# richa-batra/ParticleRobotSimulations

Hardware: AMD Instinct MI355X
Metric: particle-steps/sec at 10^6 bots; achieved HBM GB/s vs peak; 1/2/4/8-GPU ensemble (higher is better)
Workload: dtype f32

## Files before the change

include/particlebot_hip.h:

```cpp
#ifndef PARTICLEBOT_HIP_H
#define PARTICLEBOT_HIP_H

#include <stddef.h>

#include "particlebot_kernel.h"

#ifdef __cplusplus
extern "C" {
#endif

struct pbGraphicsResource;

enum { PB_RNG_COUNTER = 0, PB_RNG_XORWOW_CURAND = 1, PB_RNG_XORWOW_ROCRAND = 2 };

typedef struct pbRngState {
  unsigned d;
  unsigned v[5];
  int boxmuller_flag;
  int kind;
  float boxmuller_extra;
  float reserved[3];
} pbRngState;

int pbSetRngKind(int kind);
// ... 154 lines not shown
  int lanes_per_bot;
  int resident;
  int fast_math_ok;
  int payload;
  int rng;
  int offsets64;
  int attraction_sums;
  int dead_sum_form;
  int stream_walk;
  int tail_tiles;
  int tail_lanes;
} pbSimConfig;
int pbSimGetConfig(pbSim *sim, pbSimConfig *cfg);

typedef struct pbClockSample pbClockSample;
int pbClockSampleBegin(pbClockSample **out, double seconds);
int pbClockSampleEnd(pbClockSample *sample, double *mhz, double *seconds_sampled);

int pbSelfTest(unsigned long long div_samples, unsigned long long *sqrt_checked,
               unsigned long long *sqrt_mismatches, unsigned long long *div_checked,
               unsigned long long *div_mismatches);

int pbSelfTestHoldThreshold(float c, unsigned long long *checked, unsigned long long *mismatches);
int pbSelfTestPairGeometry(unsigned first_slice, unsigned slices, unsigned long long *checked,
                           unsigned long long *mismatches);
int pbSelfTestDivision(unsigned first_slice, unsigned slices, unsigned long long *checked,
                       unsigned long long *mismatches);

#ifdef __cplusplus
}
#endif
#endif
```

particlerobotsimulations_amd/__init__.py:

```python
import ctypes as C

import numpy as np

from . import _capi
from ._capi import SimParams, make_params, pbSimConfig, pbSimStats

__all__ = ["Sim", "Ensemble", "DeviceArray", "legacy", "SimParams", "make_params", "library_paths", "self_test"]


def self_test(div_samples=1 << 32):
    vals = [C.c_ulonglong() for _ in range(4)]
    _capi.check(_capi.lib().pbSelfTest(int(div_samples), *[C.byref(v) for v in vals]), "pbSelfTest")
    keys = ("sqrt_checked", "sqrt_mismatches", "div_checked", "div_mismatches")
    return {k: int(v.value) for k, v in zip(keys, vals)}


def self_test_hold_threshold(c):
    checked, bad = C.c_ulonglong(), C.c_ulonglong()
    _capi.check(_capi.lib().pbSelfTestHoldThreshold(float(c), C.byref(checked), C.byref(bad)), "pbSelfTestHoldThreshold")
    return {"checked": checked.value, "mismatches": bad.value}


def self_test_pair_geometry(first_slice=0, slices=64):
    checked, bad = C.c_ulonglong(), C.c_ulonglong()
    _capi.check(_capi.lib().pbSelfTestPairGeometry(int(first_slice), int(slices), C.byref(checked), C.byref(bad)),
                "pbSelfTestPairGeometry")
    return {"checked": int(checked.value), "mismatches": int(bad.value)}


def self_test_division(first_slice=0, slices=64):
    checked, bad = C.c_ulonglong(), C.c_ulonglong()
    _capi.check(_capi.lib().pbSelfTestDivision(int(first_slice), int(slices), C.byref(checked), C.byref(bad)),
                "pbSelfTestDivision")
    return {"checked": int(checked.value), "mismatches": int(bad.value)}


def force_forms():
    L = _capi.lib()
    out = []
    for i in range(L.pbForceFormCount()):
        f = _capi.pbForceForm()
        _capi.check(L.pbForceFormGet(i, C.byref(f)), "pbForceFormGet")
        out.append({k: int(getattr(f, k)) for k, _ in _capi.pbForceForm._fields_})
# ... 351 lines not shown
```

particlerobotsimulations_amd/_capi.py:

```python
import ctypes as C
import os

import numpy as np

_PKG = os.path.dirname(os.path.abspath(__file__))
LIB_DIR = os.path.join(_PKG, "lib")
HIP_SO = os.path.join(LIB_DIR, "libparticlebot_hip.so")
HOST_SO = os.path.join(LIB_DIR, "libparticlebot_host.so")

PB_MAX_OBSTACLES = 10
PB_OK = 0


class uint2(C.Structure):
    _fields_ = [("x", C.c_uint), ("y", C.c_uint)]


class float2(C.Structure):
    _fields_ = [("x", C.c_float), ("y", C.c_float)]


class SimParams(C.Structure):
    _fields_ = [
        ("gridSize", uint2), ("numCells", C.c_uint),
# ... 125 lines not shown
    "pbHostSqrtThreshold": (C.c_float, [C.c_float]),
    "pbSimSetForceVariant": (_I, [_VP, _I]),
    "pbSimSetLanesPerBot": (_I, [_VP, _I]),
    "pbSimSetTailTiles": (_I, [_VP, _I]),
    "pbForceXcdTile": (_I, [_U, _U, _U, C.POINTER(_U), C.POINTER(_U)]),
    "pbSimSetResident": (_I, [_VP, _I]),
    "pbSimGetConfig": (_I, [_VP, C.POINTER(pbSimConfig)]),
    "pbSimSetForceSums": (_I, [_VP, _I]),
    "pbSimSetStreamWalk": (_I, [_VP, _I]),
    "pbSimGetStreamWalkTrips": (_I, [_VP, C.POINTER(C.c_ulonglong), C.POINTER(C.c_ulonglong)]),
    "pbForceFormCount": (_I, []),
    "pbForceFormGet": (_I, [_I, C.POINTER(pbForceForm)]),
    "pbSimSelectForceForm": (_I, [_VP, _I]),
    "pbSimForceKernelName": (_I, [_VP, C.c_char_p, C.c_size_t]),
    "pbForceFormKernelName": (_I, [_I, _I, C.c_char_p, C.c_size_t]),
    "pbSimSetRng": (_I, [_VP, _I]),
    "pbSimGetRngStatesOf": (_I, [_VP, _U, _VP]),
    "pbSetRngKind": (_I, [_I]),
    "pbGetRngKind": (_I, []),
    "pbClockSampleBegin": (_I, [C.POINTER(_VP), C.c_double]),
    "pbClockSampleEnd": (_I, [_VP, C.POINTER(C.c_double), C.POINTER(C.c_double)]),
    "pbSelfTest": (_I, [C.c_ulonglong] + [C.POINTER(C.c_ulonglong)] * 4),
    "pbSelfTestHoldThreshold": (_I, [C.c_float, C.POINTER(C.c_ulonglong), C.POINTER(C.c_ulonglong)]),
    "pbSelfTestPairGeometry": (_I, [_U, _U, C.POINTER(C.c_ulonglong), C.POINTER(C.c_ulonglong)]),
    "pbSelfTestDivision": (_I, [_U, _U, C.POINTER(C.c_ulonglong), C.POINTER(C.c_ulonglong)]),
}

_lib = None


def lib():
    global _lib
    if _lib is not None:
        return _lib
    if not os.path.exists(HIP_SO):
        raise RuntimeError(
            f"{HIP_SO} not found: build it with `python -c 'import __graft_entry__ as g; g.build()'` "
            "(hipcc --offload-arch=gfx950).  There is no CPU fallback.")
    L = C.CDLL(HIP_SO, mode=C.RTLD_GLOBAL)
    for name, (res, args) in SYMBOLS.items():
        fn = getattr(L, name)
        fn.restype = res
        fn.argtypes = args
    _lib = L
    return L

# ... 33 lines not shown
```

particlerobotsimulations_amd/csrc/pb_device.hpp:

```cpp
#pragma once

#include <hip/hip_runtime.h>
#include <stdint.h>
#include <string.h>
#include <math.h>

#include "particlebot_kernel.h"

struct PbDevParams {
  uint32_t gridX, gridY, numCells;
  float originX, originY, cellX, cellY;
  uint32_t nCells;
  int32_t nDead;
  float gravity, spring, damping, shear, attraction, boundaryDamping, friction;
  float massFactor, frictionFactor, attractionFactor;
  float constraint, constraint_contraction;
  float light_x, light_y;
  float min_radius, max_radius, rise_period;
  int32_t Nx;
  uint32_t light_shadow, constrained_contraction, seed;
  float phase_std;
  float wallHalf;
  int32_t nobstacles;
  float x1obs[PB_MAX_OBSTACLES], x2obs[PB_MAX_OBSTACLES], y1obs[PB_MAX_OBSTACLES], y2obs[PB_MAX_OBSTACLES];
// ... 80 lines not shown
    const bool r = i < d.nobstacles;
    d.x1obs[i] = (r && p.x1obs) ? p.x1obs[i] : 0.0f;
    d.x2obs[i] = (r && p.x2obs) ? p.x2obs[i] : 0.0f;
    d.y1obs[i] = (r && p.y1obs) ? p.y1obs[i] : 0.0f;
    d.y2obs[i] = (r && p.y2obs) ? p.y2obs[i] : 0.0f;
    const bool c = i < d.n_cir;
    d.xc[i] = (c && p.x_cir_obs) ? p.x_cir_obs[i] : 0.0f;
    d.yc[i] = (c && p.y_cir_obs) ? p.y_cir_obs[i] : 0.0f;
    d.rc[i] = (c && p.r_cir_obs) ? p.r_cir_obs[i] : 0.0f;
  }
}

static inline bool pbFastMathAllowed(const PbDevParams &d) {
  auto okA = [](float a) { return a == 0.0f || (a >= 0x1p-40f && a <= 0x1p30f); };
  bool ok = okA(d.attraction) && d.wallHalf <= 4096.0f && d.wallHalf > 0.0f;
  if (d.nDead == -1) {
    const float a1 = d.attraction * d.attractionFactor;
    ok = ok && okA(a1) && okA(a1 * d.attractionFactor);
  }
  return ok;
}

static inline bool pbAttractionMagnitudeSafe(const PbDevParams &d) {
  auto okA = [](float a) { return a == 0.0f || a >= 0x1p-20f; };
  bool ok = okA(d.attraction);
  if (d.nDead == -1) {
    const float a1 = d.attraction * d.attractionFactor;
    ok = ok && okA(a1) && okA(a1 * d.attractionFactor);
  }
  return ok;
}

#include <cstddef>
static_assert(offsetof(SimParams, worldOrigin) == 16 && offsetof(SimParams, nCells) == 32 &&
                  offsetof(SimParams, nobstacles) == 144 && offsetof(SimParams, x1obs) == 152 &&
                  offsetof(SimParams, Nx) == 216 && offsetof(SimParams, max_time) == 248 &&
                  sizeof(SimParams) == 256,
              "SimParams layout drifted from the reference struct");

#define PB_DEV __device__ __forceinline__

PB_DEV float pbDot(float ax, float ay, float bx, float by) { return ax * bx + ay * by; }
PB_DEV float pbLen(float x, float y) { return sqrtf(pbDot(x, y, x, y)); }

PB_DEV int pbCellX(const PbDevParams &P, float x) { return (int)floorf((x - P.originX) / P.cellX); }
PB_DEV int pbCellY(const PbDevParams &P, float y) { return (int)floorf((y - P.originY) / P.cellY); }
PB_DEV uint32_t pbHash(const PbDevParams &P, int gx, int gy) {
  return ((uint32_t)gy & (P.gridY - 1u)) * P.gridX + ((uint32_t)gx & (P.gridX - 1u));
}

PB_DEV void pbIntegrate(const PbDevParams &P, float &px, float &py, float &vx, float &vy, float rad,
                        float dt) {
  const float W = P.wallHalf;
  px = px + vx * dt;
  py = py + vy * dt;
  if (px > W - rad) {
    px = W - rad;
    vx *= P.boundaryDamping;
  }
  if (px < -W + rad) {
    px = -W + rad;
    vx *= P.boundaryDamping;
  }
// ... 102 lines not shown
  return r;
}

PB_DEV void pbDiv2Fast(float a, float b, float d, float &qa, float &qb) {
  float r = __builtin_amdgcn_rcpf(d);
  const float e = __builtin_fmaf(-d, r, 1.0f);
  r = __builtin_fmaf(e, r, r);
  float q = a * r;
  float t = __builtin_fmaf(-d, q, a);
  qa = __builtin_fmaf(t, r, q);
  q = b * r;
  t = __builtin_fmaf(-d, q, b);
  qb = __builtin_fmaf(t, r, q);
}

PB_DEV float pbRootNewton(float x, float &s) {
  s = __builtin_amdgcn_fmed3f(__builtin_amdgcn_rsqf(x), 0.0f, 0x1.fffffep127f);
  const float h = 0.5f * s;
  float y = x * s;
  const float e = __builtin_fmaf(-y, y, x);
  return __builtin_fmaf(e, h, y);
}

PB_DEV void pbDistUnitFast(float rx, float ry, float d2, float &dist, float &nx, float &ny) {
  float s;
  const float y = pbRootNewton(d2, s);
  dist = y;
  const float er = __builtin_fmaf(-y, s, 1.0f);
  float r = __builtin_fmaf(er, s, s);
  if (__builtin_expect(__builtin_amdgcn_ballot_w64(er == 0x1p-24f) != 0ull, 0)) {
    asm volatile("; rare: reciprocal of an all-ones root, v_rcp_f32 form" ::: "memory");
    const float c = __builtin_amdgcn_rcpf(y);
    r = __builtin_fmaf(__builtin_fmaf(-y, c, 1.0f), c, c);
  }
  float q = rx * r;
  float t = __builtin_fmaf(-y, q, rx);
  nx = __builtin_fmaf(t, r, q);
  q = ry * r;
  t = __builtin_fmaf(-y, q, ry);
  ny = __builtin_fmaf(t, r, q);
}

PB_DEV bool pbTinyNonzero(float x) { return __float_as_uint(x) - 1u < 0x0F800000u - 1u; }

PB_DEV bool pbLaneFastMathOk(float x, float y) { return fabsf(x) >= 0x1p-20f && fabsf(y) >= 0x1p-20f; }

// ... 162 lines not shown
    out[k].tx = tx[k];
    out[k].ty = ty[k];
    out[k].contact = contact[k];
    if (FAST) {
      out[k].mag = pbSqrtFast(m2[k]);
      anyTiny = anyTiny || pbTinyNonzero(m2[k]);
    } else {
      out[k].mag = sqrtf(m2[k]);
    }
  }
  if (FAST) {
    if (__builtin_expect(__builtin_amdgcn_ballot_w64(anyTiny) != 0ull, 0)) {
      asm volatile("; rare: a force magnitude below 2^-48, full sqrtf" ::: "memory");
#pragma unroll
      for (int k = 0; k < K; k++) out[k].mag = sqrtf(m2[k]);
    }
  }
}

struct PbPairXY {
  float tx, ty;
};

template <bool FAST, bool WANT_A = false, class VelFetch, class PushRep>
PB_DEV PbPairXY pbPairEvalXY(const PbContactK &P, bool live, float ax, float ay, float avx, float avy, float ra,
                             float bx, float by, float rb, VelFetch velB, float attraction, float slope,
                             PushRep pushRep, float *magA = nullptr, bool *isContact = nullptr) {
  const float near1 = 0.0009f, near2 = 0.0019f, fmin_attr = 2.5f;
  const float rx = bx - ax, ry = by - ay;
  const float d2 = pbDot(rx, ry, rx, ry);
  float dist, nx, ny;
  if (FAST) {
    pbDistUnitFast(rx, ry, d2, dist, nx, ny);
  } else {
    dist = sqrtf(d2);
    nx = rx / dist;
    ny = ry / dist;
  }
  const float reach = ra + rb;
  const bool contact = dist < reach;
  const float gap = dist - reach;
  const float g2 = gap * gap;
  float tx, ty;
  if (FAST) {
    pbDiv2Fast(attraction * nx, attraction * ny, g2, tx, ty);
  } else {
    tx = attraction * nx / g2;
    ty = attraction * ny / g2;
  }
  const unsigned long long mNear = __builtin_amdgcn_ballot_w64(live) & __builtin_amdgcn_ballot_w64(gap < near2);
  if (mNear != 0ull) {
    const unsigned long long mContact = __builtin_amdgcn_ballot_w64(contact);
    if ((mNear & ~mContact) != 0ull) {
      const float band = gap < near1 ? fmin_attr : fmin_attr + slope * (gap - near1);
      tx = gap < near2 ? band * nx : tx;
      ty = gap < near2 ? band * ny : ty;
    }
    if ((mNear & mContact) != 0ull) {
      const float2 vb = velB();
      const float rvx = vb.x - avx, rvy = vb.y - avy;
      const float vn = pbDot(rvx, rvy, nx, ny);
      const float tvx = rvx - vn * nx, tvy = rvy - vn * ny;
      const float ks = -P.spring * (reach - dist);
      float cx = ks * nx;
      float cy = ks * ny;
      cx += P.damping * rvx;
      cy += P.damping * rvy;
      cx += P.shear * tvx;
      cy += P.shear * tvy;
      pushRep(contact && live, pbDot(cx, cy, cx, cy));
      tx = contact ? cx : tx;
      ty = contact ? cy : ty;
    }
  }
  if (WANT_A) {
    const float m2 = pbDot(tx, ty, tx, ty);
    float mag;
    if (FAST) {
      float s;
      mag = pbRootNewton(m2, s);
    } else {
      mag = sqrtf(m2);
    }
    *magA = mag;
    *isContact = contact;
  }
  PbPairXY r;
  r.tx = tx;
  r.ty = ty;
  return r;
}

template <bool FAST, int CAP, int STRIDE>
struct PbRepList {
  float *col;
  uint32_t off;
  PB_DEV void init(float *column) {
    col = column;
    off = 0u;
  }
  PB_DEV void flush(float &fr) {
    for (uint32_t k = 0; __builtin_amdgcn_ballot_w64(k < off) != 0ull; k += STRIDE) {
      const float m2 = col[k];
      float mag;
      if (FAST) {
        mag = pbSqrtFast(m2);
        if (__builtin_expect(__builtin_amdgcn_ballot_w64(k < off && pbTinyNonzero(m2)) != 0ull, 0)) {
          asm volatile("; rare: a contact magnitude below 2^-48, full sqrtf" ::: "memory");
// ... 307 lines not shown
```

particlerobotsimulations_amd/csrc/pb_force.hip:

```cpp
#include <cxxabi.h>

#include <algorithm>
#include <cstdlib>
#include <cstring>
#include <typeinfo>

#include "pb_engine.hpp"

#ifdef PB_TIMELINE
__device__ unsigned long long *pbTimelineBuf = nullptr;
#define PB_TL_STAMP(word)                                                                              \
  do {                                                                                                 \
    if (pbTimelineBuf && threadIdx.x == 0)                                                             \
      pbTimelineBuf[8ull * (blockIdx.y * gridDim.x + blockIdx.x) + (word)] = __builtin_amdgcn_s_memrealtime(); \
  } while (0)
#endif

#include "pb_sweep.hpp"

namespace {

template <bool PAYLOAD, bool FLAT, int L, int NB, bool BIG, bool ASUM>
__global__ __launch_bounds__(TILE, (NB == 2 ? PB_NB2_WAVES : (L == 1 && FLAT && !BIG && !PAYLOAD) ? PB_TAIL_FORM_WAVES : PB_FORCE_WAVES)) void k_force(const PbDevParams *__restrict__ params,
                                                const float4 *__restrict__ prIn, const float2 *__restrict__ velIn,
// ... 26 lines not shown
    }
  }
#ifdef PB_TIMELINE
  PB_TL_STAMP(0);
#endif
  if (l >= n) return;
  const uint32_t s = member * n + l;
  const uint32_t *__restrict__ cellS = cellSAll + (size_t)member * (P.numCells + 1u);

  const float4 me = prIn[s];
  float2 v = velIn[s];
  bool selfPayload = false;
  if (PAYLOAD) selfPayload = (orig[s] == P.nCells - 1u);
  const float att1 = selfPayload ? P.attractionFactor : 1.0f;

  PbForce F;
  F.fx = 0.0f;
  F.fy = 0.0f;
  F.fa = 0.0f;
  F.fr = 0.0f * absR[s];

  using OffT = typename std::conditional<BIG, uint64_t, uint32_t>::type;
  static_assert(ASUM || (FLAT && NB == 1), "the dead-sum form exists for the branch-free sweeps only");
  constexpr bool REPLIST = L == 1 && FLAT && NB == 1 && (!ASUM || PB_ASUM_XY);
  __shared__ float repLds[REPLIST ? (PB_REP_CAP + 1) * TILE : 1];
  float *const repCol = &repLds[REPLIST ? threadIdx.x : 0];
  auto sweep = [&](auto lanes) __attribute__((always_inline)) {
    constexpr int LS = decltype(lanes)::value;
    if (FLAT && fastOk && __all(pbLaneFastMathOk(me.x, me.y)))
      pbSweep<PAYLOAD, FLAT, true, LS, NB, OffT, ASUM>(P, prIn, velIn, cellS, 0u, s, sub, me, v, att1, F, repCol);
    else
      pbSweep<PAYLOAD, FLAT, false, LS, NB, OffT, ASUM>(P, prIn, velIn, cellS, 0u, s, sub, me, v, att1, F, repCol);
  };
  if (TAILABLE && tailWg)
    sweep(std::integral_constant<int, TAILABLE ? PB_TAIL_LANES : L>{});
  else
    sweep(std::integral_constant<int, L>{});
  pbObstacles(P, me.x, me.y, v.x, v.y, me.z, F);
  pbFrictionAndKick(P, selfPayload, F.fx, F.fy, dt, v.x, v.y);

  float4 out = me;
  if (fuse) {
    if (doRadiusNext) out.z = pbActuate(P, me.z, phase[s], dead[s], F.fa, F.fr, timeNext, dt);
    pbIntegrate(P, out.x, out.y, v.x, v.y, out.z, dt);
  }
  if (sub == 0) {
    prOut[s] = out;
// ... 15 lines not shown
  if (S->tailTiles >= 0) return std::min((uint32_t)S->tailTiles, perXcd);
  if (S->cuCount == 0) {
    int cus = 0;
    if (hipDeviceGetAttribute(&cus, hipDeviceAttributeMultiprocessorCount, S->device) != hipSuccess || cus <= 0) cus = 256;
    S->cuCount = (uint32_t)cus;
  }
  const uint32_t cusPerXcd = std::max(S->cuCount / 8u, 1u);
  const uint32_t wgPerCu = PB_TAIL_FORM_WAVES * 4u / (TILE / 64u);
  return perXcd >= cusPerXcd * wgPerCu ? cusPerXcd : 0u;
}

template <bool PAYLOAD, bool FLAT, int L, bool BIG, bool ASUM>
void launchForceT(pbSim *S, bool fuse, int c, int o, float dt, float tNext, int doRadiusNext) {
  const uint32_t tiles = cdiv(S->n, TILE / L);
  const uint32_t perXcd = ((L == 1 || S->xcdTilesAll) && tiles >= 64u) ? cdiv(tiles, 8u) : 0u;
  constexpr int NB = (FLAT && L == 1 && !BIG && ASUM) ? PB_THROUGHPUT_NB : 1;
  const uint32_t tail = (FLAT && L == 1 && NB == 1 && !BIG && perXcd) ? pbTailTiles(S, perXcd) : 0u;
  dim3 grid(perXcd ? (perXcd + tail * (PB_TAIL_LANES - 1)) * 8u : tiles, S->nsims);
  uint32_t memberTiles = tail;
  if (S->xcdMembers && !perXcd && S->nsims >= 8u) {
    memberTiles = tiles;
    grid = dim3(cdiv(S->nsims, 8u) * 8u * tiles, 1u);
  }
  const bool magNeeded = ASUM && FLAT && L == 1 && PB_ASUM_XY;
  const int fastOk = (S->variant >= 2 && S->fastOk && (!magNeeded || S->magOk)) ? 1 : 0;
  hipLaunchKernelGGL((k_force<PAYLOAD, FLAT, L, NB, BIG, ASUM>), grid, dim3(TILE), S->debugLdsBytes, S->stream, S->dP,
                     S->pr[c], S->vel[c], S->cellS, S->absR[c], S->n, perXcd, memberTiles, S->nsims, dt, fastOk, S->pr[o],
                     S->vel[o], S->phase[c], S->dead[c], S->absA[c], S->orig[c], tNext, doRadiusNext, (int)fuse);
}

template <bool PAYLOAD, bool FLAT, int L, bool BIG, bool ASUM>
std::string forceNameT() {
  constexpr int NB = (FLAT && L == 1 && !BIG && ASUM) ? PB_THROUGHPUT_NB : 1;
  auto b = [](bool v) { return std::string(v ? "true" : "false"); };
  return "k_force<" + b(PAYLOAD) + ", " + b(FLAT) + ", " + std::to_string(L) + ", " + std::to_string(NB) + ", " + b(BIG) +
         ", " + b(ASUM) + ">" + pbKernelArgs(typeid(&k_force<PAYLOAD, FLAT, L, NB, BIG, ASUM>).name());
}

using LaunchFn = void (*)(pbSim *, bool, int, int, float, float, int);
using NameFn = std::string (*)();
struct FormRow {
  pbForceForm form;
  LaunchFn launch[2];
  NameFn name[2];
};
#define PB_FORM(FL, LL, AS, BG)                                                        \
  {{FL, LL, AS, BG}, {launchForceT<false, (FL) != 0, LL, (BG) != 0, (AS) != 0>,        \
// ... 140 lines not shown
```

particlerobotsimulations_amd/csrc/pb_resident.hip:

```cpp
#include "pb_engine.hpp"
#include "pb_sweep.hpp"

namespace {

template <bool PAYLOAD, bool FASTOK, int L, bool ASUM = true>
__global__ __launch_bounds__(1024) void k_resident(const PbDevParams *__restrict__ params, float4 *__restrict__ pr,
                                                   float2 *__restrict__ vel, const float *__restrict__ phase,
                                                   const int *__restrict__ dead, float *__restrict__ absA,
                                                   float *__restrict__ absR, const uint32_t *__restrict__ orig,
                                                   const uint32_t *__restrict__ cellSAll, uint32_t n, float dt,
                                                   float time0, int nsteps, int lightWave) {
  constexpr int CAP = 1024 / L;
  __shared__ float4 sPr[2][CAP + 1];
  __shared__ float2 sVel[2][CAP + 1];
  constexpr bool REPLIST = L == 1 && (!ASUM || PB_ASUM_XY);
  __shared__ float repLds[REPLIST ? (PB_REP_CAP + 1) * 1024 : 1];
  static_assert(sizeof(sPr) + sizeof(sVel) + sizeof(repLds) <= 160 * 1024, "k_resident: LDS beyond one CU");
  float *const repCol = &repLds[REPLIST ? threadIdx.x : 0];
  const PbDevParams &P = params[blockIdx.x];
  const uint32_t l = threadIdx.x / L, sub = threadIdx.x % L;
  const bool active = l < n;
  const uint32_t base = blockIdx.x * n;
  const uint32_t s = base + (active ? l : 0u);
  const uint32_t *__restrict__ cellS = cellSAll + (size_t)blockIdx.x * (P.numCells + 1u);

  float4 me = pr[s];
  float2 v = vel[s];
  const float ph = phase[s];
  const int dd = dead[s];
  float fa = absA[s], fr = absR[s];
  bool selfPayload = false;
  if (PAYLOAD) selfPayload = (orig[s] == P.nCells - 1u);
  const float att1 = selfPayload ? P.attractionFactor : 1.0f;

  PbSegCache segCache;
  segCache.gx = segCache.gy = (int)0x80000000;
  segCache.m = 0;
  float t = time0;
// ... 69 lines not shown

namespace {

template <bool PAYLOAD, bool FASTOK, bool ASUM>
void launchResidentT(pbSim *S, float dt, float t0, int m, int lightWave) {
  const int c = S->cur;
  const int L = residentLanes(S->n);
  const dim3 grid(S->nsims), block(cdiv(S->n * (uint32_t)L, 64u) * 64u);
#define PB_RES(LL)                                                                                      \
  hipLaunchKernelGGL((k_resident<PAYLOAD, FASTOK, LL, ASUM>), grid, block, 0, S->stream, S->dP, S->pr[c], S->vel[c], \
                     S->phase[c], S->dead[c], S->absA[c], S->absR[c], S->orig[c], S->cellS, S->n, dt, t0, m,   \
                     lightWave)
  if (L == 8) PB_RES(8);
  else if (L == 4) PB_RES(4);
  else if (L == 2) PB_RES(2);
  else PB_RES(1);
#undef PB_RES
}

}

void pbLaunchResident(pbSim *S, float dt, float t0, int m, int lightWave) {
  const bool asum = attractionSumsKept(S);
  const bool magNeeded = asum && residentLanes(S->n) == 1 && PB_ASUM_XY;
  const bool fast = S->variant >= 2 && S->fastOk && (!magNeeded || S->magOk);
#define PB_RESL(PL, FA)                                                   \
  do {                                                                    \
    if (asum) launchResidentT<PL, FA, true>(S, dt, t0, m, lightWave);     \
    else launchResidentT<PL, FA, false>(S, dt, t0, m, lightWave);         \
  } while (0)
  if (S->payload) {
    if (fast) PB_RESL(true, true);
    else PB_RESL(true, false);
  } else {
    if (fast) PB_RESL(false, true);
    else PB_RESL(false, false);
  }
#undef PB_RESL
}
```

particlerobotsimulations_amd/csrc/pb_selftest.hip:

```cpp
#include "pb_engine.hpp"

namespace {

__global__ __launch_bounds__(256) void k_selftest_sqrt(unsigned long long *__restrict__ mismatches,
                                                       unsigned long long *__restrict__ checked) {
  const uint32_t base = (blockIdx.x * 256u + threadIdx.x) * 16u;
  uint32_t bad = 0, seen = 0;
  for (uint32_t k = 0; k < 16u; k++) {
    const uint32_t bits = base + k;
    const bool inDomain = bits == 0u || (bits >= 0x0F800000u && bits <= 0x7F800000u);
    if (!inDomain) continue;
    const float x = __uint_as_float(bits);
    seen++;
    if (__float_as_uint(pbSqrtFast(x)) != __float_as_uint(sqrtf(x))) bad++;
    if (bits != 0x7F800000u) {
      float dist, nx, ny;
      pbDistUnitFast(0.0f, 0.0f, x, dist, nx, ny);
      if (__float_as_uint(dist) != __float_as_uint(sqrtf(x))) bad++;
    }
  }
  if (bad) atomicAdd(mismatches, (unsigned long long)bad);
  if (seen) atomicAdd(checked, (unsigned long long)seen);
}

__global__ __launch_bounds__(256) void k_selftest_hold(float c, float T, unsigned long long *__restrict__ mismatches,
                                                       unsigned long long *__restrict__ checked) {
  const uint32_t base = (blockIdx.x * 256u + threadIdx.x) * 16u;
  uint32_t bad = 0;
  for (uint32_t k = 0; k < 16u; k++) {
    const float x = __uint_as_float(base + k);
    if ((sqrtf(x) < c) != (x < T)) bad++;
  }
  if (bad) atomicAdd(mismatches, (unsigned long long)bad);
  if (threadIdx.x == 0) atomicAdd(checked, 256ull * 16ull);
}

PB_DEV bool pbDivNoScale(uint32_t nb, uint32_t db) {
  const int en = (int)((nb >> 23) & 255u), ed = (int)((db >> 23) & 255u);
  if ((nb & 0x7FFFFFFFu) == 0u) return (nb == 0u) && ed >= 1 && ed <= 252;
  return ed >= 1 && ed <= 252 && en >= 27 && en <= 254 && (en - ed) < 96 && (en - ed) > -125;
}

// ... 129 lines not shown
  PB_TRY(hipMemcpy(h, d, sizeof(h), hipMemcpyDeviceToHost));
  PB_TRY(hipFree(d));
  if (sqrt_checked) *sqrt_checked = h[0];
  if (sqrt_mismatches) *sqrt_mismatches = h[1];
  if (div_checked) *div_checked = h[2];
  if (div_mismatches) *div_mismatches = h[3];
  return PB_OK;
}

int pbSelfTestHoldThreshold(float c, unsigned long long *checked, unsigned long long *mismatches) {
  unsigned long long *d = nullptr;
  PB_TRY(hipMalloc((void **)&d, 2 * sizeof(unsigned long long)));
  PB_TRY(hipMemset(d, 0, 2 * sizeof(unsigned long long)));
  hipLaunchKernelGGL(k_selftest_hold, dim3(1u << 19), dim3(256), 0, 0, c, pbSqrtThreshold(c), d + 1, d + 0);
  PB_TRY(hipGetLastError());
  unsigned long long h[2];
  PB_TRY(hipMemcpy(h, d, sizeof(h), hipMemcpyDeviceToHost));
  PB_TRY(hipFree(d));
  if (checked) *checked = h[0];
  if (mismatches) *mismatches = h[1];
  return PB_OK;
}

int pbSelfTestPairGeometry(unsigned first_slice, unsigned slices, unsigned long long *checked,
                           unsigned long long *mismatches) {
  if (first_slice >= 64u || slices == 0u || first_slice + slices > 64u) return PB_ERR_ARG;
  unsigned long long *d = nullptr;
  PB_TRY(hipMalloc((void **)&d, 2 * sizeof(unsigned long long)));
  PB_TRY(hipMemset(d, 0, 2 * sizeof(unsigned long long)));
  const uint32_t perSlice = (1u << 24) / 64u;
  for (unsigned sl = first_slice; sl < first_slice + slices; sl++)
    hipLaunchKernelGGL(k_selftest_geom_exhaustive, dim3(perSlice * 8u / 256u), dim3(256), 0, 0, sl * perSlice, d + 1, d + 0);
  PB_TRY(hipGetLastError());
  unsigned long long h[2];
  PB_TRY(hipMemcpy(h, d, sizeof(h), hipMemcpyDeviceToHost));
  PB_TRY(hipFree(d));
  if (checked) *checked = h[0];
  if (mismatches) *mismatches = h[1];
  return PB_OK;
}

int pbSelfTestDivision(unsigned first_slice, unsigned slices, unsigned long long *checked,
                       unsigned long long *mismatches) {
  if (first_slice >= 64u || slices == 0u || first_slice + slices > 64u) return PB_ERR_ARG;
  unsigned long long *d = nullptr;
  PB_TRY(hipMalloc((void **)&d, 2 * sizeof(unsigned long long)));
// ... 52 lines not shown
```

particlerobotsimulations_amd/csrc/pb_sweep.hpp:

```cpp
#pragma once

#include <type_traits>

#include "pb_device.hpp"
#include "pb_engine.hpp"

#ifndef PB_FORCE_WAVES
#define PB_FORCE_WAVES 1
#endif
#ifndef PB_NB2_WAVES
#define PB_NB2_WAVES 8
#endif
#ifndef PB_THROUGHPUT_NB
#define PB_THROUGHPUT_NB 1
#endif
#ifndef PB_PREFETCH_DEPTH
#define PB_PREFETCH_DEPTH 1
#endif
#ifndef PB_REP_CAP
#define PB_REP_CAP 8
#endif

#ifndef PB_TAIL_FORM_WAVES
#define PB_TAIL_FORM_WAVES 8
#endif
#ifndef PB_ASUM_XY
#define PB_ASUM_XY 1
#endif
#ifndef PB_LAZY_VEL
#define PB_LAZY_VEL 1
#endif
#ifndef PB_SWEEP_EXPERIMENT
#define PB_SWEEP_EXPERIMENT 0
#endif
#ifndef PB_TL_STAMP
#define PB_TL_STAMP(word) do { } while (0)
#endif

template <int L>
__device__ __forceinline__ float pbShr1(float v) {
  if (L <= 16)
    return __int_as_float(__builtin_amdgcn_update_dpp(0, __float_as_int(v), 0x111 , 0xF, 0xF, false));
  return __int_as_float(__builtin_amdgcn_update_dpp(0, __float_as_int(v), 0x138 , 0xF, 0xF, false));
}
template <int L>
__device__ __forceinline__ float pbGroupLast(float v) {
  if (L == 64) return __int_as_float(__builtin_amdgcn_readlane(__float_as_int(v), 63));
  constexpr int PAT = ((L - 1) << 5) | (0x1F & ~(L - 1));
  return __int_as_float(__builtin_amdgcn_ds_swizzle(__float_as_int(v), PAT));
}
template <int L>
__device__ __forceinline__ void pbGroupSum(bool live, const PbPairTerm &t, PbForce &F) {
  const float tx = live ? t.tx : 0.0f, ty = live ? t.ty : 0.0f;
  const float ta = (live && !t.contact) ? t.mag : 0.0f, tr = (live && t.contact) ? t.mag : 0.0f;
  float ax = F.fx + tx, ay = F.fy + ty, aa = F.fa + ta, ar = F.fr + tr;
#pragma unroll
// ... 146 lines not shown
                float mag;
                if (FAST) {
                  mag = pbSqrtFast(m2);
                  if (__builtin_expect(__builtin_amdgcn_ballot_w64(mine && pbTinyNonzero(m2)) != 0ull, 0)) {
                    asm volatile("; rare: a contact magnitude below 2^-48, full sqrtf" ::: "memory");
                    mag = sqrtf(m2);
                  }
                } else {
                  mag = sqrtf(m2);
                }
                pbGroupSum1<L>(mine ? mag : 0.0f, F.fr);
              });
          pbGroupSumXY<L>(live[0], t, F);
        }
      }
    };
    if (__all(nseg == 1)) run(std::false_type{});
    else run(std::true_type{});
    return;
  }
  if (FLAT && NB == 1) {
    const char *const prBytes = (const char *)&prIn[0];
    const char *const velBytes = (const char *)&velIn[0];
    const OffT selfOff = (OffT)s * 16u;
    auto at = [&](OffT off) __attribute__((always_inline)) { return *(const float4 *)(prBytes + off); };
    auto vat = [&](OffT off) __attribute__((always_inline)) { return *(const float2 *)(velBytes + (off >> 1)); };
    constexpr bool REPL = !ASUM || PB_ASUM_XY;
    PbRepList<FAST, PB_REP_CAP, REPSTRIDE> rep;
    if (REPL) rep.init(repCol);
#if PB_SWEEP_EXPERIMENT >= 2
    auto atI = [&](OffT off, int imm) __attribute__((always_inline)) {
      float4 q = me;
      asm volatile("" : "+v"(q.x), "+v"(q.y), "+v"(q.z) : "v"(off));
      q.x += 0.3f;
      return q;
    };
#else
    auto atI = [&](OffT off, int imm) __attribute__((always_inline)) {
      return *(const float4 *)(prBytes + (uint64_t)off + imm);
    };
#endif
#if PB_SWEEP_EXPERIMENT >= 1
    auto vatI = [&](OffT hoff, int imm) __attribute__((always_inline)) {
      float2 w = v;
      asm volatile("" : "+v"(w.x), "+v"(w.y) : "v"(hoff));
      return w;
    };
#else
    auto vatI = [&](OffT hoff, int imm) __attribute__((always_inline)) {
      return *(const float2 *)(velBytes + (uint64_t)hoff + imm);
    };
#endif
    const OffT selfOff16 = selfOff + 16u;
    auto one = [&](const float4 &q, auto velOf, bool isLive) __attribute__((always_inline)) {
      const bool live[1] = {isLive};
      const float bx[1] = {q.x}, by[1] = {q.y}, rb[1] = {q.z};
      const float A[1] = {PAYLOAD ? attraction0 * q.w * att1 : attraction0};
      const float K[1] = {PAYLOAD ? pbBandSlope(A[0]) : slope0};
      if (ASUM && !PB_ASUM_XY) {
        PbPairTerm t[1];
        pbPairEvalK<FAST, 1>(CK, live, me.x, me.y, v.x, v.y, me.z, bx, by, rb, A, K, [&](int) { return velOf(); }, t);
        pbPairAdd(live[0], t[0], F);
      } else if (ASUM) {
        float magA;
        bool contact;
        const PbPairXY t = pbPairEvalXY<FAST, true>(CK, live[0], me.x, me.y, v.x, v.y, me.z, q.x, q.y, q.z, velOf, A[0],
                                                    K[0], [&](bool mine, float m2) { rep.push(mine, m2, F.fr); }, &magA,
                                                    &contact);
        if (live[0]) {
          asm volatile("");
          F.fx += t.tx;
          F.fy += t.ty;
          if (!contact) F.fa += magA;
        }
      } else {
        const PbPairXY t = pbPairEvalXY<FAST>(CK, live[0], me.x, me.y, v.x, v.y, me.z, q.x, q.y, q.z, velOf, A[0],
                                              K[0], [&](bool mine, float m2) { rep.push(mine, m2, F.fr); });
        if (live[0]) {
          asm volatile("");
          F.fx += t.tx;
          F.fy += t.ty;
        }
      }
    };
    auto bounds = [&](int si, OffT &lo, OffT &hi) __attribute__((always_inline)) {
      lo = hi = selfOff;
      if (si < 10) {
        const uint32_t row = ((uint32_t)(gy + (si >> 1) - 2) & (P.gridY - 1u)) << P.gridXLog2;
        lo = (OffT)(cellS[row + ((si & 1) ? 0u : mx0)] - base) * 16u;
        hi = (OffT)(cellS[row + ((si & 1) ? 5u - first : mx0 + first)] - base) * 16u;
      }
    };
    const int stride = nseg == 1 ? 2 : 1;
    OffT loA, hiA, loB, hiB;
    bounds(0, loA, hiA);
    bounds(stride, loB, hiB);
    float4 qA = at(loA);
    float2 vA = vat(loA);
    PB_TL_STAMP(4);
#pragma unroll 1
    for (int si = 0; si < 10; si += stride) {
      if (si == 4) PB_TL_STAMP(5);
      const OffT lo = loA, end = hiA;
      float4 q0 = qA;
      float2 v0 = vA;
      loA = loB;
      hiA = hiB;
      qA = at(loA);
      vA = vat(loA);
      bounds(si + 2 * stride, loB, hiB);
      if (lo < end) {
#if PB_PREFETCH_DEPTH == 2
        OffT off = lo, hoff = lo >> 1;
        const OffT endm16 = end - 16u, endm32 = end > 32u ? end - 32u : 0u, endm48 = end > 48u ? end - 48u : 0u;
        float4 q1 = atI(off, 16);
        for (;;) {
          const float4 q2 = atI(off, 32);
          one(q0, [&]() { return vatI(hoff, 0); }, off != selfOff);
          if (off >= endm16) break;
          q0 = atI(off, 48);
          one(q1, [&]() { return vatI(hoff, 8); }, off != selfOff - 16u);
          if (off >= endm32) break;
          q1 = atI(off, 64);
          one(q2, [&]() { return vatI(hoff, 16); }, off != selfOff - 32u);
          if (off >= endm48) break;
          off += 48u;
          hoff += 24u;
        }
#else
        OffT off = lo, hoff = lo >> 1;
        const OffT endm = end - 16u;
#if PB_LAZY_VEL
        (void)v0;
        for (;;) {
          const float4 q1 = atI(off, 16);
          one(q0, [&]() { return vatI(hoff, 0); }, off != selfOff);
          if (off >= endm) break;
          off += 32u;
          hoff += 16u;
          q0 = atI(off, 0);
          one(q1, [&]() { return vatI(hoff, -8); }, off != selfOff16);
          if (off >= end) break;
        }
#else
        for (;;) {
          const float4 q1 = atI(off, 16);
          const float2 v1 = vatI(hoff, 8);
          one(q0, [&]() { return v0; }, off != selfOff);
          if (off >= endm) break;
          off += 32u;
          hoff += 16u;
          q0 = atI(off, 0);
          v0 = vatI(hoff, 0);
          one(q1, [&]() { return v1; }, off != selfOff16);
          if (off >= end) break;
        }
#endif
#endif
      }
    }
    if (REPL) rep.flush(F.fr);
    return;
  }
  if (FLAT && NB == 2) {
    const char *const prBytes = (const char *)&prIn[0];
    const char *const velBytes = (const char *)&velIn[0];
    const uint32_t selfOff = s * 16u;
    auto at = [&](uint32_t off) __attribute__((always_inline)) { return *(const float4 *)(prBytes + off); };
    auto vat = [&](uint32_t off) __attribute__((always_inline)) { return *(const float2 *)(velBytes + (off >> 1)); };
    auto two = [&](const float4 &qa, const float2 &va, const float4 &qb, const float2 &vb, uint32_t off,
                   uint32_t end) __attribute__((always_inline)) {
      const bool live[2] = {off != selfOff, (off + 16u != selfOff) && (off + 16u < end)};
      const float bx[2] = {qa.x, qb.x}, by[2] = {qa.y, qb.y}, rb[2] = {qa.z, qb.z};
      const float A[2] = {PAYLOAD ? attraction0 * qa.w * att1 : attraction0,
                          PAYLOAD ? attraction0 * qb.w * att1 : attraction0};
      const float K[2] = {PAYLOAD ? pbBandSlope(A[0]) : slope0, PAYLOAD ? pbBandSlope(A[1]) : slope0};
      PbPairTerm t[2];
      pbPairEvalK<FAST, 2>(CK, live, me.x, me.y, v.x, v.y, me.z, bx, by, rb, A, K,
                           [&](int k) { return k == 0 ? va : vb; }, t);
      pbPairAdd(live[0], t[0], F);
      pbPairAdd(live[1], t[1], F);
    };
    auto bounds = [&](int si, uint32_t &lo, uint32_t &hi) __attribute__((always_inline)) {
      lo = hi = selfOff;
// ... 103 lines not shown
```

Baseline: 10.78 billion.

## Split neighbor sweep around self slot and streamline attraction magnitude root

The flat single-neighbor sweep now cuts the cell range containing the bot itself into two pieces, so the inner loop no longer tests every neighbor against the self offset. The attraction magnitude uses a new Newton root built on the hardware reciprocal square root, accumulated inside the pair evaluation, and contact is computed only where the near band needs it. The change also removes the dead experiment, prefetch-depth and non-XY attraction-sum branches, makes the repulsion list unconditional, and adds a self-test that checks the new root bit-exactly against sqrtf. The attraction-safety check now rejects a zero attraction, which may push some configurations onto the slow path, and the split adds extra outer-loop trips.

Result: faster. 10.95 billion (median of 6 runs) (+1.6%).

```diff
diff --git a/include/particlebot_hip.h b/include/particlebot_hip.h
--- a/include/particlebot_hip.h
+++ b/include/particlebot_hip.h
@@ -200,6 +200,7 @@
                unsigned long long *div_mismatches);
 
 int pbSelfTestHoldThreshold(float c, unsigned long long *checked, unsigned long long *mismatches);
+int pbSelfTestMagnitudeRoot(unsigned long long *checked, unsigned long long *mismatches);
 int pbSelfTestPairGeometry(unsigned first_slice, unsigned slices, unsigned long long *checked,
                            unsigned long long *mismatches);
 int pbSelfTestDivision(unsigned first_slice, unsigned slices, unsigned long long *checked,
diff --git a/particlerobotsimulations_amd/__init__.py b/particlerobotsimulations_amd/__init__.py
--- a/particlerobotsimulations_amd/__init__.py
+++ b/particlerobotsimulations_amd/__init__.py
@@ -19,6 +19,12 @@
     checked, bad = C.c_ulonglong(), C.c_ulonglong()
     _capi.check(_capi.lib().pbSelfTestHoldThreshold(float(c), C.byref(checked), C.byref(bad)), "pbSelfTestHoldThreshold")
     return {"checked": checked.value, "mismatches": bad.value}
+
+
+def self_test_magnitude_root():
+    checked, bad = C.c_ulonglong(), C.c_ulonglong()
+    _capi.check(_capi.lib().pbSelfTestMagnitudeRoot(C.byref(checked), C.byref(bad)), "pbSelfTestMagnitudeRoot")
+    return {"checked": int(checked.value), "mismatches": int(bad.value)}
 
 
 def self_test_pair_geometry(first_slice=0, slices=64):
diff --git a/particlerobotsimulations_amd/_capi.py b/particlerobotsimulations_amd/_capi.py
--- a/particlerobotsimulations_amd/_capi.py
+++ b/particlerobotsimulations_amd/_capi.py
@@ -171,6 +171,7 @@
     "pbClockSampleEnd": (_I, [_VP, C.POINTER(C.c_double), C.POINTER(C.c_double)]),
     "pbSelfTest": (_I, [C.c_ulonglong] + [C.POINTER(C.c_ulonglong)] * 4),
     "pbSelfTestHoldThreshold": (_I, [C.c_float, C.POINTER(C.c_ulonglong), C.POINTER(C.c_ulonglong)]),
+    "pbSelfTestMagnitudeRoot": (_I, [C.POINTER(C.c_ulonglong), C.POINTER(C.c_ulonglong)]),
     "pbSelfTestPairGeometry": (_I, [_U, _U, C.POINTER(C.c_ulonglong), C.POINTER(C.c_ulonglong)]),
     "pbSelfTestDivision": (_I, [_U, _U, C.POINTER(C.c_ulonglong), C.POINTER(C.c_ulonglong)]),
 }
diff --git a/particlerobotsimulations_amd/csrc/pb_device.hpp b/particlerobotsimulations_amd/csrc/pb_device.hpp
--- a/particlerobotsimulations_amd/csrc/pb_device.hpp
+++ b/particlerobotsimulations_amd/csrc/pb_device.hpp
@@ -126,7 +126,7 @@
 }
 
 static inline bool pbAttractionMagnitudeSafe(const PbDevParams &d) {
-  auto okA = [](float a) { return a == 0.0f || a >= 0x1p-20f; };
+  auto okA = [](float a) { return a >= 0x1p-20f; };
   bool ok = okA(d.attraction);
   if (d.nDead == -1) {
     const float a1 = d.attraction * d.attractionFactor;
@@ -143,6 +143,10 @@
               "SimParams layout drifted from the reference struct");
 
 #define PB_DEV __device__ __forceinline__
+
+#ifndef PB_TRIP_TRIM
+#define PB_TRIP_TRIM 5
+#endif
 
 PB_DEV float pbDot(float ax, float ay, float bx, float by) { return ax * bx + ay * by; }
 PB_DEV float pbLen(float x, float y) { return sqrtf(pbDot(x, y, x, y)); }
@@ -291,6 +295,19 @@
   return __builtin_fmaf(e, h, y);
 }
 
+PB_DEV float pbRootNewtonPositive(float x) {
+#if PB_TRIP_TRIM & 4
+  const float s = __builtin_amdgcn_rsqf(x);
+  const float h = 0.5f * s;
+  const float y = x * s;
+  const float e = __builtin_fmaf(-y, y, x);
+  return __builtin_fmaf(e, h, y);
+#else
+  float s;
+  return pbRootNewton(x, s);
+#endif
+}
+
 PB_DEV void pbDistUnitFast(float rx, float ry, float d2, float &dist, float &nx, float &ny) {
   float s;
   const float y = pbRootNewton(d2, s);
@@ -499,10 +516,16 @@
   float tx, ty;
 };
 
+template <bool FAST>
+PB_DEV float pbAttractionMagnitude(float tx, float ty) {
+  const float m2 = pbDot(tx, ty, tx, ty);
+  return FAST ? pbRootNewtonPositive(m2) : sqrtf(m2);
+}
+
 template <bool FAST, bool WANT_A = false, class VelFetch, class PushRep>
 PB_DEV PbPairXY pbPairEvalXY(const PbContactK &P, bool live, float ax, float ay, float avx, float avy, float ra,
                              float bx, float by, float rb, VelFetch velB, float attraction, float slope,
-                             PushRep pushRep, float *magA = nullptr, bool *isContact = nullptr) {
+                             PushRep pushRep, float *fa = nullptr) {
   const float near1 = 0.0009f, near2 = 0.0019f, fmin_attr = 2.5f;
   const float rx = bx - ax, ry = by - ay;
   const float d2 = pbDot(rx, ry, rx, ry);
@@ -515,7 +538,6 @@
     ny = ry / dist;
   }
   const float reach = ra + rb;
-  const bool contact = dist < reach;
   const float gap = dist - reach;
   const float g2 = gap * gap;
   float tx, ty;
@@ -527,6 +549,7 @@
   }
   const unsigned long long mNear = __builtin_amdgcn_ballot_w64(live) & __builtin_amdgcn_ballot_w64(gap < near2);
   if (mNear != 0ull) {
+    const bool contact = dist < reach;
     const unsigned long long mContact = __builtin_amdgcn_ballot_w64(contact);
     if ((mNear & ~mContact) != 0ull) {
       const float band = gap < near1 ? fmin_attr : fmin_attr + slope * (gap - near1);
@@ -551,16 +574,8 @@
     }
   }
   if (WANT_A) {
-    const float m2 = pbDot(tx, ty, tx, ty);
-    float mag;
-    if (FAST) {
-      float s;
-      mag = pbRootNewton(m2, s);
-    } else {
-      mag = sqrtf(m2);
-    }
-    *magA = mag;
-    *isContact = contact;
+    const float mag = pbAttractionMagnitude<FAST>(tx, ty);
+    if (live && !(dist < reach)) *fa += mag;
   }
   PbPairXY r;
   r.tx = tx;
diff --git a/particlerobotsimulations_amd/csrc/pb_force.hip b/particlerobotsimulations_amd/csrc/pb_force.hip
--- a/particlerobotsimulations_amd/csrc/pb_force.hip
+++ b/particlerobotsimulations_amd/csrc/pb_force.hip
@@ -72,7 +72,7 @@
 
   using OffT = typename std::conditional<BIG, uint64_t, uint32_t>::type;
   static_assert(ASUM || (FLAT && NB == 1), "the dead-sum form exists for the branch-free sweeps only");
-  constexpr bool REPLIST = L == 1 && FLAT && NB == 1 && (!ASUM || PB_ASUM_XY);
+  constexpr bool REPLIST = L == 1 && FLAT && NB == 1;
   __shared__ float repLds[REPLIST ? (PB_REP_CAP + 1) * TILE : 1];
   float *const repCol = &repLds[REPLIST ? threadIdx.x : 0];
   auto sweep = [&](auto lanes) __attribute__((always_inline)) {
@@ -134,7 +134,7 @@
     memberTiles = tiles;
     grid = dim3(cdiv(S->nsims, 8u) * 8u * tiles, 1u);
   }
-  const bool magNeeded = ASUM && FLAT && L == 1 && PB_ASUM_XY;
+  const bool magNeeded = ASUM && FLAT && L == 1;
   const int fastOk = (S->variant >= 2 && S->fastOk && (!magNeeded || S->magOk)) ? 1 : 0;
   hipLaunchKernelGGL((k_force<PAYLOAD, FLAT, L, NB, BIG, ASUM>), grid, dim3(TILE), S->debugLdsBytes, S->stream, S->dP,
                      S->pr[c], S->vel[c], S->cellS, S->absR[c], S->n, perXcd, memberTiles, S->nsims, dt, fastOk, S->pr[o],
diff --git a/particlerobotsimulations_amd/csrc/pb_resident.hip b/particlerobotsimulations_amd/csrc/pb_resident.hip
--- a/particlerobotsimulations_amd/csrc/pb_resident.hip
+++ b/particlerobotsimulations_amd/csrc/pb_resident.hip
@@ -13,7 +13,7 @@
   constexpr int CAP = 1024 / L;
   __shared__ float4 sPr[2][CAP + 1];
   __shared__ float2 sVel[2][CAP + 1];
-  constexpr bool REPLIST = L == 1 && (!ASUM || PB_ASUM_XY);
+  constexpr bool REPLIST = L == 1;
   __shared__ float repLds[REPLIST ? (PB_REP_CAP + 1) * 1024 : 1];
   static_assert(sizeof(sPr) + sizeof(sVel) + sizeof(repLds) <= 160 * 1024, "k_resident: LDS beyond one CU");
   float *const repCol = &repLds[REPLIST ? threadIdx.x : 0];
@@ -129,7 +129,7 @@
 
 void pbLaunchResident(pbSim *S, float dt, float t0, int m, int lightWave) {
   const bool asum = attractionSumsKept(S);
-  const bool magNeeded = asum && residentLanes(S->n) == 1 && PB_ASUM_XY;
+  const bool magNeeded = asum && residentLanes(S->n) == 1;
   const bool fast = S->variant >= 2 && S->fastOk && (!magNeeded || S->magOk);
 #define PB_RESL(PL, FA)                                                   \
   do {                                                                    \
diff --git a/particlerobotsimulations_amd/csrc/pb_selftest.hip b/particlerobotsimulations_amd/csrc/pb_selftest.hip
--- a/particlerobotsimulations_amd/csrc/pb_selftest.hip
+++ b/particlerobotsimulations_amd/csrc/pb_selftest.hip
@@ -18,6 +18,21 @@
       pbDistUnitFast(0.0f, 0.0f, x, dist, nx, ny);
       if (__float_as_uint(dist) != __float_as_uint(sqrtf(x))) bad++;
     }
+  }
+  if (bad) atomicAdd(mismatches, (unsigned long long)bad);
+  if (seen) atomicAdd(checked, (unsigned long long)seen);
+}
+
+__global__ __launch_bounds__(256) void k_selftest_magroot(unsigned long long *__restrict__ mismatches,
+                                                          unsigned long long *__restrict__ checked) {
+  const uint32_t base = (blockIdx.x * 256u + threadIdx.x) * 16u;
+  uint32_t bad = 0, seen = 0;
+  for (uint32_t k = 0; k < 16u; k++) {
+    const uint32_t bits = base + k;
+    if (bits < 0x0F800000u || bits >= 0x7F7FFFFFu) continue;
+    const float x = __uint_as_float(bits);
+    seen++;
+    if (__float_as_uint(pbRootNewtonPositive(x)) != __float_as_uint(sqrtf(x))) bad++;
   }
   if (bad) atomicAdd(mismatches, (unsigned long long)bad);
   if (seen) atomicAdd(checked, (unsigned long long)seen);
@@ -193,6 +208,20 @@
   return PB_OK;
 }
 
+int pbSelfTestMagnitudeRoot(unsigned long long *checked, unsigned long long *mismatches) {
+  unsigned long long *d = nullptr;
+  PB_TRY(hipMalloc((void **)&d, 2 * sizeof(unsigned long long)));
+  PB_TRY(hipMemset(d, 0, 2 * sizeof(unsigned long long)));
+  hipLaunchKernelGGL(k_selftest_magroot, dim3(1u << 19), dim3(256), 0, 0, d + 1, d + 0);
+  PB_TRY(hipGetLastError());
+  unsigned long long h[2];
+  PB_TRY(hipMemcpy(h, d, sizeof(h), hipMemcpyDeviceToHost));
+  PB_TRY(hipFree(d));
+  if (checked) *checked = h[0];
+  if (mismatches) *mismatches = h[1];
+  return PB_OK;
+}
+
 int pbSelfTestPairGeometry(unsigned first_slice, unsigned slices, unsigned long long *checked,
                            unsigned long long *mismatches) {
   if (first_slice >= 64u || slices == 0u || first_slice + slices > 64u) return PB_ERR_ARG;
diff --git a/particlerobotsimulations_amd/csrc/pb_sweep.hpp b/particlerobotsimulations_amd/csrc/pb_sweep.hpp
--- a/particlerobotsimulations_amd/csrc/pb_sweep.hpp
+++ b/particlerobotsimulations_amd/csrc/pb_sweep.hpp
@@ -14,24 +14,12 @@
 #ifndef PB_THROUGHPUT_NB
 #define PB_THROUGHPUT_NB 1
 #endif
-#ifndef PB_PREFETCH_DEPTH
-#define PB_PREFETCH_DEPTH 1
-#endif
 #ifndef PB_REP_CAP
 #define PB_REP_CAP 8
 #endif
 
 #ifndef PB_TAIL_FORM_WAVES
 #define PB_TAIL_FORM_WAVES 8
-#endif
-#ifndef PB_ASUM_XY
-#define PB_ASUM_XY 1
-#endif
-#ifndef PB_LAZY_VEL
-#define PB_LAZY_VEL 1
-#endif
-#ifndef PB_SWEEP_EXPERIMENT
-#define PB_SWEEP_EXPERIMENT 0
 #endif
 #ifndef PB_TL_STAMP
 #define PB_TL_STAMP(word) do { } while (0)
@@ -224,65 +212,30 @@
   if (FLAT && NB == 1) {
     const char *const prBytes = (const char *)&prIn[0];
     const char *const velBytes = (const char *)&velIn[0];
+    constexpr bool SPLIT = (PB_TRIP_TRIM & 1) != 0;
     const OffT selfOff = (OffT)s * 16u;
+    const OffT selfOff16 = selfOff + 16u;
     auto at = [&](OffT off) __attribute__((always_inline)) { return *(const float4 *)(prBytes + off); };
-    auto vat = [&](OffT off) __attribute__((always_inline)) { return *(const float2 *)(velBytes + (off >> 1)); };
-    constexpr bool REPL = !ASUM || PB_ASUM_XY;
     PbRepList<FAST, PB_REP_CAP, REPSTRIDE> rep;
-    if (REPL) rep.init(repCol);
-#if PB_SWEEP_EXPERIMENT >= 2
-    auto atI = [&](OffT off, int imm) __attribute__((always_inline)) {
-      float4 q = me;
-      asm volatile("" : "+v"(q.x), "+v"(q.y), "+v"(q.z) : "v"(off));
-      q.x += 0.3f;
-      return q;
-    };
-#else
+    rep.init(repCol);
     auto atI = [&](OffT off, int imm) __attribute__((always_inline)) {
       return *(const float4 *)(prBytes + (uint64_t)off + imm);
     };
-#endif
-#if PB_SWEEP_EXPERIMENT >= 1
-    auto vatI = [&](OffT hoff, int imm) __attribute__((always_inline)) {
-      float2 w = v;
-      asm volatile("" : "+v"(w.x), "+v"(w.y) : "v"(hoff));
-      return w;
-    };
-#else
     auto vatI = [&](OffT hoff, int imm) __attribute__((always_inline)) {
       return *(const float2 *)(velBytes + (uint64_t)hoff + imm);
     };
-#endif
-    const OffT selfOff16 = selfOff + 16u;
-    auto one = [&](const float4 &q, auto velOf, bool isLive) __attribute__((always_inline)) {
-      const bool live[1] = {isLive};
-      const float bx[1] = {q.x}, by[1] = {q.y}, rb[1] = {q.z};
-      const float A[1] = {PAYLOAD ? attraction0 * q.w * att1 : attraction0};
-      const float K[1] = {PAYLOAD ? pbBandSlope(A[0]) : slope0};
-      if (ASUM && !PB_ASUM_XY) {
-        PbPairTerm t[1];
-        pbPairEvalK<FAST, 1>(CK, live, me.x, me.y, v.x, v.y, me.z, bx, by, rb, A, K, [&](int) { return velOf(); }, t);
-        pbPairAdd(live[0], t[0], F);
-      } else if (ASUM) {
-        float magA;
-        bool contact;
-        const PbPairXY t = pbPairEvalXY<FAST, true>(CK, live[0], me.x, me.y, v.x, v.y, me.z, q.x, q.y, q.z, velOf, A[0],
-                                                    K[0], [&](bool mine, float m2) { rep.push(mine, m2, F.fr); }, &magA,
-                                                    &contact);
-        if (live[0]) {
-          asm volatile("");
-          F.fx += t.tx;
-          F.fy += t.ty;
-          if (!contact) F.fa += magA;
-        }
-      } else {
-        const PbPairXY t = pbPairEvalXY<FAST>(CK, live[0], me.x, me.y, v.x, v.y, me.z, q.x, q.y, q.z, velOf, A[0],
-                                              K[0], [&](bool mine, float m2) { rep.push(mine, m2, F.fr); });
-        if (live[0]) {
-          asm volatile("");
-          F.fx += t.tx;
-          F.fy += t.ty;
-        }
+    auto one = [&](const float4 &q, auto velOf, bool live) __attribute__((always_inline)) {
+      const float A = PAYLOAD ? attraction0 * q.w * att1 : attraction0;
+      const float K = PAYLOAD ? pbBandSlope(A) : slope0;
+      const PbPairXY t = pbPairEvalXY<FAST, ASUM>(CK, live, me.x, me.y, v.x, v.y, me.z, q.x, q.y, q.z, velOf, A, K,
+                                                  [&](bool mine, float m2) { rep.push(mine, m2, F.fr); }, &F.fa);
+      if (SPLIT) {
+        F.fx += t.tx;
+        F.fy += t.ty;
+      } else if (live) {
+        asm volatile("");
+        F.fx += t.tx;
+        F.fy += t.ty;
       }
     };
     auto bounds = [&](int si, OffT &lo, OffT &hi) __attribute__((always_inline)) {
@@ -298,70 +251,35 @@
     bounds(0, loA, hiA);
     bounds(stride, loB, hiB);
     float4 qA = at(loA);
-    float2 vA = vat(loA);
     PB_TL_STAMP(4);
 #pragma unroll 1
-    for (int si = 0; si < 10; si += stride) {
+    for (int si = 0; si < 10;) {
       if (si == 4) PB_TL_STAMP(5);
-      const OffT lo = loA, end = hiA;
+      const OffT lo = loA;
+      const bool cut = SPLIT && (OffT)(selfOff - lo) < (OffT)(hiA - lo);
+      const OffT end = cut ? selfOff : hiA;
       float4 q0 = qA;
-      float2 v0 = vA;
-      loA = loB;
-      hiA = hiB;
+      loA = cut ? selfOff16 : loB;
+      hiA = cut ? hiA : hiB;
       qA = at(loA);
-      vA = vat(loA);
-      bounds(si + 2 * stride, loB, hiB);
+      if (!cut) bounds(si + 2 * stride, loB, hiB);
+      si += cut ? 0 : stride;
       if (lo < end) {
-#if PB_PREFETCH_DEPTH == 2
-        OffT off = lo, hoff = lo >> 1;
-        const OffT endm16 = end - 16u, endm32 = end > 32u ? end - 32u : 0u, endm48 = end > 48u ? end - 48u : 0u;
-        float4 q1 = atI(off, 16);
-        for (;;) {
-          const float4 q2 = atI(off, 32);
-          one(q0, [&]() { return vatI(hoff, 0); }, off != selfOff);
-          if (off >= endm16) break;
-          q0 = atI(off, 48);
-          one(q1, [&]() { return vatI(hoff, 8); }, off != selfOff - 16u);
-          if (off >= endm32) break;
-          q1 = atI(off, 64);
-          one(q2, [&]() { return vatI(hoff, 16); }, off != selfOff - 32u);
-          if (off >= endm48) break;
-          off += 48u;
-          hoff += 24u;
-        }
-#else
         OffT off = lo, hoff = lo >> 1;
         const OffT endm = end - 16u;
-#if PB_LAZY_VEL
-        (void)v0;
         for (;;) {
           const float4 q1 = atI(off, 16);
-          one(q0, [&]() { return vatI(hoff, 0); }, off != selfOff);
+          one(q0, [&]() { return vatI(hoff, 0); }, SPLIT || off != selfOff);
           if (off >= endm) break;
           off += 32u;
           hoff += 16u;
           q0 = atI(off, 0);
-          one(q1, [&]() { return vatI(hoff, -8); }, off != selfOff16);
+          one(q1, [&]() { return vatI(hoff, -8); }, SPLIT || off != selfOff16);
           if (off >= end) break;
         }
-#else
-        for (;;) {
-          const float4 q1 = atI(off, 16);
-          const float2 v1 = vatI(hoff, 8);
-          one(q0, [&]() { return v0; }, off != selfOff);
-          if (off >= endm) break;
-          off += 32u;
-          hoff += 16u;
-          q0 = atI(off, 0);
-          v0 = vatI(hoff, 0);
-          one(q1, [&]() { return v1; }, off != selfOff16);
-          if (off >= end) break;
-        }
-#endif
-#endif
       }
     }
-    if (REPL) rep.flush(F.fr);
+    rep.flush(F.fr);
     return;
   }
   if (FLAT && NB == 2) {
```
